# JonathanLehner/korali

Measured on AMD Instinct MI355X. Metric: CMA-ES generations/sec + samples/sec, 128-dim Rosenbrock λ=4096, 1→8 GPUs, higher is better.
Workload: dtype f64; 1 GPU; C2: CMA-ES, 128-dim negative Rosenbrock, lambda=4096, mu=2048 Logarithmic, x0=0, sigma0=1, seed 1337; one experiment per GPU; population=4096, variables=128, covariance_update=exact, parallelism=replicas1

## Files before the change

### korali_amd/csrc/kg_cmaes.hip

```cpp
#include <cmath>
#include <cstdio>
#include <cstdlib>
#include <cstring>
#include <map>
#include <string>
#include <tuple>
#include <vector>

#include "../../include/korali_amd.h"
#include "kg_common.hpp"
#include "kg_chains.hpp"
#include "kg_eigen.hpp"
#include "kg_rng.hpp"
#include <chrono>

namespace kg {


struct CmaesScalars {
  double sigma, trace, effectiveMu, cumulativeCovariance, sigmaCumulationFactor, dampFactor, chiSquareNumber;
  double psNorm, bestEverValue, previousBestEverValue, previousBestValue, currentBestValue;
  double currentMinStd, currentMaxStd, maxDiagC, minDiagC, minEig, maxEig;
  double infeasibleSampleCount, bestValidSample, modelEvaluationCount, hsig, eigenFailures;
  double ccov1, ccovmu;
// ... 1141 lines not shown
    tile[r][tx] = t;
  }
  if (k0 == 0 && ty == 0 && d0 + tx < N) prevMean[d0 + tx] = md;
  __syncthreads();
  for (int r = ty; r < RP_T; r += 8) {
    const int d = d0 + r, k = k0 + tx;
    if (d < N && k < mu) Tt[(size_t)d * mu + k] = tile[tx][r];
  }
  if (__syncthreads_or(!ok) && threadIdx.x == 0) atomicOr(&sc->rmuOutOfRange, 1u);
  if (blockIdx.x || blockIdx.y) return;
  __shared__ int flag;
  if (threadIdx.x == 0) {
    const unsigned i0 = sidx[0];
    sc->bestValidSample = (double)i0;
    sc->previousBestValue = sc->currentBestValue;
    sc->currentBestValue = F[i0];
    flag = (sc->currentBestValue > sc->bestEverValue || gen == 1) ? 1 : 0;
    sc->bestFlag = (unsigned)flag;
    if (flag) {
      sc->previousBestEverValue = sc->bestEverValue;
      sc->bestEverValue = sc->currentBestValue;
    }
  }
  __syncthreads();
  const unsigned i0 = sidx[0];
  for (int d = threadIdx.x; d < N; d += blockDim.x) {
    const double v = X[(size_t)i0 * N + d];
    currBestVars[d] = v;
    if (flag) bestEverVars[d] = v;
  }
}

constexpr int RS_U = 8;
__global__ void __launch_bounds__(256) k_rank_select(int lam, int N, int mu, unsigned long long gen,
                                                     const double *__restrict__ F, unsigned *__restrict__ out,
                                                     const double *__restrict__ X, const double *__restrict__ w,
                                                     const double *__restrict__ mean, double *__restrict__ prevMean,
                                                     double *__restrict__ Y, double *__restrict__ currBestVars,
                                                     double *__restrict__ bestEverVars, CmaesScalars *sc,
                                                     double *__restrict__ Yc, double *__restrict__ Tt) {
  extern __shared__ __attribute__((aligned(16))) double rk[];
  __shared__ unsigned part[16][17];
  __shared__ unsigned rank_s[16];
  __shared__ int flag;
  const int row = threadIdx.x >> 4, c = threadIdx.x & 15;
  const int is = blockIdx.x * 16 + row;
  double xv[RS_U], mv[RS_U];
#pragma unroll
  for (int u = 0; u < RS_U; u++) {
    const int d = c + 16 * u;
    xv[u] = (is < lam && d < N) ? X[(size_t)is * N + d] : 0.0;
    mv[u] = d < N ? mean[d] : 0.0;
  }
  const double effMu = sc->effectiveMu, ca = N + 1.3, cb = N + 2.0;
  const double ccov1 = 2.0 / (ca * ca + effMu);
  double ccovmu = 2.0 * (effMu - 2. + 1. / effMu) / (cb * cb + effMu);
  if (1.0 - ccov1 < ccovmu) ccovmu = 1.0 - ccov1;
  for (int q0 = threadIdx.x; q0 < lam; q0 += 8 * blockDim.x) {
    double v[8];
#pragma unroll
    for (int u = 0; u < 8; u++) v[u] = (q0 + u * (int)blockDim.x < lam) ? F[q0 + u * blockDim.x] : 0.0;
#pragma unroll
    for (int u = 0; u < 8; u++)
      if (q0 + u * (int)blockDim.x < lam) rk[q0 + u * blockDim.x] = v[u];
  }
  if (blockIdx.x == 0)
// ... 5 lines not shown
    const double ki = (i < lam) ? rk[i] : 0.0;
    const int per = (lam + 15) / 16, j0 = p * per, j1 = min(lam, j0 + per);
    unsigned cnt = 0;
    int j = j0;
    for (; j + 8 <= j1; j += 8) {
      double kj[8];
#pragma unroll
      for (int u = 0; u < 8; u++) kj[u] = rk[j + u];
#pragma unroll
      for (int u = 0; u < 8; u++) cnt += (kj[u] > ki || (kj[u] == ki && j + u < i)) ? 1u : 0u;
    }
    for (; j < j1; j++) {
      const double kj = rk[j];
      cnt += (kj > ki || (kj == ki && j < i)) ? 1u : 0u;
    }
    part[p][li] = cnt;
  }
  __syncthreads();
  if (threadIdx.x < 16) {
    unsigned r = 0;
    for (int q = 0; q < 16; q++) r += part[q][threadIdx.x];
    rank_s[threadIdx.x] = r;
    if (blockIdx.x * 16 + (int)threadIdx.x < lam) out[r] = (unsigned)(blockIdx.x * 16 + threadIdx.x);
  }
  __syncthreads();
  const unsigned r = rank_s[row];
  const bool sel = is < lam && r < (unsigned)mu;
  bool ok = true;
  if (sel) {
    const double cw = ccovmu * w[r];
    auto put = [&](int d, double x, double m) {
      Y[(size_t)r * N + d] = x;
      const double yc = x - m;
      Yc[(size_t)r * N + d] = yc;
      const double t = cw * yc;
      Tt[(size_t)d * mu + r] = t;
      ok = ok && rmu_in_range(yc) && rmu_in_range(t);
    };
#pragma unroll
    for (int u = 0; u < RS_U; u++)
      if (c + 16 * u < N) put(c + 16 * u, xv[u], mv[u]);
    for (int d = c + 16 * RS_U; d < N; d += 16) put(d, X[(size_t)is * N + d], mean[d]);
  }
  if (__syncthreads_or(!ok) && threadIdx.x == 0) atomicOr(&sc->rmuOutOfRange, 1u);
  const bool best = is < lam && r == 0u;
  if (!__syncthreads_or(best)) return;
  if (best && c == 0) {
    sc->bestValidSample = (double)is;
    sc->previousBestValue = sc->currentBestValue;
    sc->currentBestValue = rk[is];
    const int fl = (sc->currentBestValue > sc->bestEverValue || gen == 1) ? 1 : 0;
    flag = fl;
    sc->bestFlag = (unsigned)fl;
    if (fl) {
      sc->previousBestEverValue = sc->bestEverValue;
      sc->bestEverValue = sc->currentBestValue;
    }
  }
  __syncthreads();
  if (best) {
    const int fl = flag;
#pragma unroll
    for (int u = 0; u < RS_U; u++) {
      const int d = c + 16 * u;
      if (d < N) {
        currBestVars[d] = xv[u];
        if (fl) bestEverVars[d] = xv[u];
      }
    }
// ... 241 lines not shown
  const bool active = wid == 0 && d < N && e < N && e <= d && (!diagonal || e == d);
  const double ccov1 = sc->ccov1, ccovmu = sc->ccovmu, cc = sc->cumulativeCovariance;
  const int hsig = (int)sc->hsig;
  const double s2 = sc->sigma * sc->sigma;
  double c = 0.0;
  if (active) {
    const double Cde = C[(size_t)d * N + e];
    c = (1 - ccov1 - ccovmu) * Cde + ccov1 * (pc[d] * pc[e] + (1 - hsig) * cc * (2. - cc) * Cde);
  }
  const int ex = (int)((__double_as_longlong(s2) >> 52) & 0x7ff) - 1023;
  if (__builtin_amdgcn_readfirstlane((int)(sc->rmuOutOfRange == 0u && ex >= -100 && ex <= 100)))
    c = ax3_run<true>(c, Yc, Tt, N, mu, d0, e0, wid, lane, s2, 1.0 / s2, Q);
  else
    c = ax3_run<false>(c, Yc, Tt, N, mu, d0, e0, wid, lane, s2, 0.0, Q);
  if (active) {
    C[(size_t)d * N + e] = c;
    if (e < d) C[(size_t)e * N + d] = c;
  }
}

#ifndef KG_AR_TC
#define KG_AR_TC 4
#endif
constexpr int AR_TC = KG_AR_TC, AR_NT = 64 * AR_TC, AR_K = 256, AR_KS = AR_K + 2, AR_TU = 4 * AR_K / AR_NT,
              AR_YU = AR_TC * AR_K / AR_NT;
static_assert(AR_TC == 4 || AR_TC == 8, "4 x 4 or 4 x 8 tiles");
__host__ __device__ inline int ar_row_blocks(int N) { return (N + 3) / 4; }
__host__ __device__ inline int ar_col_blocks_upto(int rb) { return (4 * rb + 3) / AR_TC + 1; }
int ar_tiles(int N) {
  int t = 0;
  for (int rb = 0; rb < ar_row_blocks(N); rb++) t += std::min(ar_col_blocks_upto(rb), (N + AR_TC - 1) / AR_TC);
  return t;
}
template <bool kMarkstein>
__device__ __forceinline__ double ar_run(double acc, int N, int mu, int d0, int e0, int dl, int el,
                                         const double *__restrict__ Yc, const double *__restrict__ Tt, double s2,
                                         double (*Ts)[4][AR_KS], double (*Ys)[AR_TC][AR_KS]) {
  const int tid = threadIdx.x, j = tid & 15;
  const double y = kMarkstein ? 1.0 / s2 : 0.0;
  double tv[AR_TU], yv[AR_YU];
  auto load = [&](int k0) {
#pragma unroll
    for (int u = 0; u < AR_TU; u++) {
      const int q = tid + AR_NT * u, r = q / AR_K;
      int kq = q % AR_K;
      asm volatile("" : "+v"(kq));
      const int k = k0 + kq;
      tv[u] = (d0 + r < N && k < mu) ? Tt[(size_t)(d0 + r) * mu + k] : 0.0;
    }
#pragma unroll
    for (int u = 0; u < AR_YU; u++) {
      const int q = tid + AR_NT * u, k = k0 + q / AR_TC, c = q % AR_TC;
      yv[u] = (k < mu && e0 + c < N) ? Yc[(size_t)k * N + e0 + c] : 0.0;
    }
  };
  auto store = [&](int b) {
#pragma unroll
    for (int u = 0; u < AR_TU; u++) {
      const int q = tid + AR_NT * u;
      int kq = q % AR_K;
      asm volatile("" : "+v"(kq));
      Ts[b][q / AR_K][kq] = tv[u];
    }
#pragma unroll
    for (int u = 0; u < AR_YU; u++) {
      const int q = tid + AR_NT * u;
      Ys[b][q % AR_TC][q / AR_TC] = yv[u];
    }
  };
  load(0);
  store(0);
  __syncthreads();
  for (int k0 = 0, b = 0; k0 < mu; k0 += AR_K, b ^= 1) {
    const bool more = k0 + AR_K < mu;
    if (more) load(k0 + AR_K);
    const int gn = (min(AR_K, mu - k0) + 15) >> 4;
    for (int g = 0; g < gn; g++) {
      const double pr = Ts[b][dl][16 * g + j] * Ys[b][el][16 * g + j];
      double q;
      if (kMarkstein) {
        const double q0 = pr * y;
        const double r = __builtin_fma(-q0, s2, pr);
        q = __builtin_fma(r, y, q0);
      } else {
        q = pr / s2;
      }
      acc = chains::kc_row16(acc, q);
    }
    if (more) store(b ^ 1);
    __syncthreads();
  }
  return acc;
}
__global__ void __launch_bounds__(AR_NT) k_adaptC_row(int N, int mu, int diagonal, const double *__restrict__ Yc,
                                                    const double *__restrict__ Tt, const double *__restrict__ pc,
                                                    double *C, const CmaesScalars *__restrict__ sc, int tbase,
                                                    double *__restrict__ pack) {
  __shared__ double Ts[2][4][AR_KS];
  __shared__ double Ys[2][AR_TC][AR_KS];
  const int tid = threadIdx.x, lane = tid & 63, wid = tid >> 6;
  const int row = lane >> 4, j = lane & 15;
  int t = blockIdx.x + tbase, rb = 0;
  const int ncb = (N + AR_TC - 1) / AR_TC;
  for (;; rb++) {
    const int c = min(ar_col_blocks_upto(rb), ncb);
    if (t < c) break;
    t -= c;
  }
  const int d0 = 4 * rb, e0 = AR_TC * t;
  const int dl = wid / (AR_TC / 4), el = 4 * (wid % (AR_TC / 4)) + row;
  const int d = d0 + dl, e = e0 + el;
  const bool active = d < N && e < N && e <= d && (!diagonal || e == d);
  const double ccov1 = sc->ccov1, ccovmu = sc->ccovmu, cc = sc->cumulativeCovariance;
  const int hsig = (int)sc->hsig;
  const double s2 = sc->sigma * sc->sigma;
  double acc = 0.0;
  if (active) {
    const double Cde = C[(size_t)d * N + e];
    acc = (1 - ccov1 - ccovmu) * Cde + ccov1 * (pc[d] * pc[e] + (1 - hsig) * cc * (2. - cc) * Cde);
  }
  const int ex = (int)((__double_as_longlong(s2) >> 52) & 0x7ff) - 1023;
  if (__builtin_amdgcn_readfirstlane((int)(sc->rmuOutOfRange == 0u && ex >= -100 && ex <= 100)))
    acc = ar_run<true>(acc, N, mu, d0, e0, dl, el, Yc, Tt, s2, Ts, Ys);
  else
    acc = ar_run<false>(acc, N, mu, d0, e0, dl, el, Yc, Tt, s2, Ts, Ys);
  if (pack) {
    if (j == 0 && d < N && e <= d) pack[(size_t)d * (d + 1) / 2 + e] = active ? acc : C[(size_t)d * N + e];
    return;
  }
  if (active && j == 0) {
    C[(size_t)d * N + e] = acc;
    if (e < d) C[(size_t)e * N + d] = acc;
  }
}

#ifndef KG_AL_K
#define KG_AL_K 64
#endif
constexpr int AL_T = 16, AL_K = KG_AL_K, AL_KP = AL_K + 2;
static_assert(AL_K % 2 == 0, "two terms per ds_read_b128");
__host__ __device__ inline int al_blocks(int N) { return (N + AL_T - 1) / AL_T; }
int al_tiles(int N) { return al_blocks(N) * (al_blocks(N) + 1) / 2; }
template <bool kMarkstein>
__device__ __forceinline__ void al_run(int N, int mu, int diagonal, const double *__restrict__ Yc,
                                       const double *__restrict__ Tt, const double *__restrict__ pc, double *C,
                                       const CmaesScalars *__restrict__ sc, int tbase, double *__restrict__ pack,
                                       double (*Ts)[AL_T][AL_KP], double (*Ys)[AL_T][AL_KP]) {
  const int tid = threadIdx.x, dl = tid >> 4, el = tid & 15;
  int t = blockIdx.x + tbase, bd = 0;
  while (t > bd) t -= ++bd;
  const int d0 = AL_T * bd, e0 = AL_T * t;
  const int d = d0 + dl, e = e0 + el;
  const bool active = d < N && e <= d && (!diagonal || e == d);
  const double ccov1 = sc->ccov1, ccovmu = sc->ccovmu, cc = sc->cumulativeCovariance;
  const int hsig = (int)sc->hsig;
  const double s2 = sc->sigma * sc->sigma, y = kMarkstein ? 1.0 / s2 : 0.0;
  double acc = 0.0;
  if (active) {
// ... 172 lines not shown
        const bool ok = e < MN_D * MN2_R && i < mu && c < nd;
        wv[u] = ok ? w[i] : 0.0;
        yv[u] = ok ? Y[(size_t)i * N + d0 + c] : 0.0;
      }
#pragma unroll
      for (int u = 0; u < 8; u++) {
        const int e = e0 + u * nt, r = e >> 3, c = e & 7;
        if (e < MN_D * MN2_R) b[(size_t)c * MN2_RS + r] = wv[u] * yv[u];
      }
    }
  };
  stage(0, tid, 256);
  __syncthreads();
  double acc = 0.0;
  const int c = lane < nd ? lane : 0;
  for (int ch = 0; ch < nchunks; ch++) {
    if (wid == 0) {
      const int rn = min(MN2_R, mu - ch * MN2_R);
      const double *b = pbuf + (size_t)(ch & 1) * MN_D * MN2_RS + (size_t)c * MN2_RS;
      acc = chains::kc_add(acc, lds_addr(b), __builtin_amdgcn_readfirstlane((unsigned)(rn + 15) >> 4));
    } else if (ch + 1 < nchunks) {
      stage(ch + 1, tid - 64, 192);
    }
    __syncthreads();
  }
  if (wid == 0 && lane < nd) {
    const int d = d0 + lane;
    const double prev = prevMean[d];
    mean[d] = acc;
    meanUpdate[d] = (acc - prev) / sc->sigma;
  }
}

constexpr int MR_K = 256, MR_KS = MR_K + 2, MR_U = MR_K * 16 / 256;
constexpr int PR_T = 1024;
template <bool kWait>
__device__ void paths3_body(int N, unsigned long long gen, const double *__restrict__ B, const double *__restrict__ D,
                            const double *meanUpdate, double *auxBDZ, double *ps, double *pc, CmaesScalars *sc,
                            unsigned *arrived, unsigned target);
template <bool kPaths>
__global__ void __launch_bounds__(kPaths ? PR_T : 256)
    k_mean3(int N, int mu, const double *__restrict__ Y, const double *__restrict__ w, double *mean,
            const double *__restrict__ prevMean, double *meanUpdate, CmaesScalars *sc, unsigned long long gen,
            const double *__restrict__ B, const double *__restrict__ D, double *auxBDZ, double *ps, double *pc,
            unsigned *arrived, unsigned target) {
  if (kPaths) {
    if (blockIdx.x == gridDim.x - 1) {
      paths3_body<true>(N, gen, B, D, meanUpdate, auxBDZ, ps, pc, sc, arrived, target);
      return;
    }
    if (threadIdx.x >= 256) return;
  }
  __shared__ double ys[2][16][MR_KS];
  __shared__ double ws[2][MR_K];
  const int tid = threadIdx.x, lane = tid & 63, wid = tid >> 6;
  const int row = lane >> 4, j = lane & 15, dl = 4 * wid + row;
  const int d0 = blockIdx.x * 16;
  const int nch = (mu + MR_K - 1) / MR_K;
  const double pmd = (j == 0 && d0 + dl < N) ? prevMean[d0 + dl] : 0.0, sig = sc->sigma;
  double ld[MR_U], wl = 0.0;
  auto load = [&](int ch) {
#pragma unroll
    for (int u = 0; u < MR_U; u++) {
      const int q = tid + 256 * u, k = q >> 4, c = q & 15, i = ch * MR_K + k;
      ld[u] = (i < mu && d0 + c < N) ? Y[(size_t)i * N + d0 + c] : 0.0;
    }
    const int i = ch * MR_K + tid;
    wl = (tid < MR_K && i < mu) ? w[i] : 0.0;
  };
  auto store = [&](int b) {
#pragma unroll
    for (int u = 0; u < MR_U; u++) {
      const int q = tid + 256 * u, k = q >> 4, c = q & 15;
      ys[b][c][k] = ld[u];
    }
    if (tid < MR_K) ws[b][tid] = wl;
  };
  load(0);
  store(0);
  __syncthreads();
  double acc = 0.0;
  for (int ch = 0; ch < nch; ch++) {
    const int b = ch & 1;
    if (ch + 1 < nch) load(ch + 1);
    const int gn = min(MR_K, mu - ch * MR_K + 15) >> 4;
    for (int g = 0; g < gn; g++) {
      const double q = ws[b][16 * g + j] * ys[b][dl][16 * g + j];
      acc = chains::kc_row16(acc, q);
    }
    if (ch + 1 < nch) store(b ^ 1);
    __syncthreads();
  }
  const int d = d0 + dl;
  if (j == 0 && d < N) {
    mean[d] = acc;
    meanUpdate[d] = (acc - pmd) / sig;
    if (kPaths) __builtin_amdgcn_fence(__ATOMIC_RELEASE, "agent");
  }
  if (kPaths) {
    __syncthreads();
    if (tid == 0) __hip_atomic_fetch_add(arrived, 1u, __ATOMIC_RELAXED, __HIP_MEMORY_SCOPE_AGENT);
  }
}

template <bool kWait>
__device__ __forceinline__ void paths3_body(int N, unsigned long long gen, const double *__restrict__ B,
                                            const double *__restrict__ D, const double *meanUpdate, double *auxBDZ,
                                            double *ps, double *pc, CmaesScalars *sc, unsigned *arrived,
                                            unsigned target) {
  __shared__ double mu_s[128 + 16], aux_s[128 + 16], pn_s[128 + 16];
  __shared__ int hs;
  const int tid = threadIdx.x, lane = tid & 63, wid = tid >> 6;
  const int row = lane >> 4, j = lane & 15;
  const double cs = sc->sigmaCumulationFactor, effMu = sc->effectiveMu, cc = sc->cumulativeCovariance;
  const double chi = sc->chiSquareNumber, hpGen = sc->hsigPowGen, hpCs = sc->hsigPowCs, hp = sc->hsigPow;
  const double pcq = tid < N ? pc[tid] : 0.0;
  double muq = (!kWait && tid < N) ? meanUpdate[tid] : 0.0;
  double Dd[2], psd[2];
#pragma unroll
  for (int p = 0; p < 2; p++) {
    const int d = 64 * p + 4 * wid + row;
    Dd[p] = (j == 0 && d < N) ? D[d] : 1.0;
    psd[p] = (j == 0 && d < N) ? ps[d] : 0.0;
  }
// ... 826 lines not shown
  double *Yc = nullptr, *Tt = nullptr;
  double *dzT = nullptr;
  size_t dzTRows = 0;
  int trW = 0;
  EigenSolver eig;
  int *infeas = nullptr, *assign = nullptr;
  int *selEnd = nullptr;
  unsigned long long *blockEnd = nullptr, *usedBlocks = nullptr;
  bool stateDirty = true;
  size_t resamplingRounds = 0;
  bool mirrored = false;
  double *G = nullptr;
  bool hasDiscrete = false;
  double *gran = nullptr, *mask = nullptr, *maskSigma = nullptr, *ubuf = nullptr, *dzero = nullptr;
  unsigned long long *uused = nullptr;
  size_t ucap = 0;
  size_t blocks = 0;
  int kslices = 8;
  int shards = 1, shardRank = 0, r0 = 0, r1 = 0;
  bool replSample = false;
  int *kidx = nullptr, *shardCnt = nullptr;
  double *part = nullptr;
  int *shardPos = nullptr, *shardCounts = nullptr;
  double *rows = nullptr, *covPack = nullptr;
  size_t rowsCap = 0;
  int rowBlock = -1;
  unsigned long long *eigTrace = nullptr;
  TermSummary *summary = nullptr, *summaryDev = nullptr;
  unsigned long long updates = 0;
  bool sampleBegun = false;
  bool consumePending = false;
  bool fusedSel = true, earlyPub = true;
  bool fusedDraw = true;
  unsigned *meanArrived = nullptr;
  unsigned meanTarget = 0;
  MtStream normal, uniform;
  bool profile = false;
  std::vector<std::tuple<std::string, hipEvent_t, hipEvent_t>> pending;
  std::map<std::string, hipEvent_t> openMarks;
  std::map<std::string, std::pair<double, size_t>> prof;
};

namespace {

struct Stage {
  kg_cmaes_s *h;
  std::string name;
  hipEvent_t a = nullptr, b = nullptr;
  hipStream_t s;
  Stage(kg_cmaes_s *h_, const char *n, hipStream_t on = nullptr) : h(h_), name(n), s(on ? on : h_->stream) {
    if (h->profile) {
      (void)hipEventCreate(&a);
      (void)hipEventCreate(&b);
      (void)hipEventRecord(a, s);
    }
  }
  ~Stage() {
    if (h->profile) {
      (void)hipEventRecord(b, s);
      h->pending.emplace_back(name, a, b);
    }
  }
};

int flush_consume(kg_cmaes_s *h) {
  if (!h->consumePending) return 0;
// ... 322 lines not shown
          dalloc_q(&h->pairCnt, h->nc * (size_t)L) | dalloc_q(&h->listDev, L);
    h->cEval.assign(h->nc * (size_t)L, 0.0);
    h->cInd.assign(h->nc * (size_t)L, 0.0);
    h->cCnt.assign(L, 0.0);
    h->vBounds.assign(h->nc, 0.0);
    h->bestCEval.assign(h->nc, 0.0);
  }
  rc |= dalloc_q(&h->kidx, h->muMax) | dalloc_q(&h->shardCnt, 1) | dalloc_q(&h->part, 2 * (size_t)N + (size_t)(nt * (nt + 1) / 2) * 256);
  if (cfg->shard_count >= 1 && cfg->cov_mode != KG_COV_MFMA) {
    h->rowsCap = h->replSample ? 0 : (size_t)std::min(h->muMax, L / h->shards);
    rc |= dalloc_q(&h->shardPos, h->muMax) | dalloc_q(&h->shardCounts, h->shards + 1) |
          dalloc_q(&h->covPack, (size_t)N * (N + 1) / 2);
    if (h->rowsCap) rc |= dalloc_q(&h->rows, (size_t)h->shards * h->rowsCap * N);
  }
  if (!rc && hipStreamSynchronize(nullptr) != hipSuccess) {
    set_error("kg_cmaes_create: zero fills of the device buffers failed");
    rc = 1;
  }
  if (rc) {
    delete h;
    return 1;
  }
  clk.mark("buffers");
  if (getenv("KORALI_AMD_TRACE_EIGEN")) rc |= dalloc(&h->eigTrace, 32 + 8 * (size_t)std::max(N, 128));
  if (host_alloc(&h->summary, sizeof(TermSummary), hipHostMallocCoherent | hipHostMallocMapped) != hipSuccess ||
      hipHostGetDevicePointer((void **)&h->summaryDev, h->summary, 0) != hipSuccess) {
    delete h;
    KG_CHECK(false, "hipHostMalloc of the termination summary failed");
  }
  memset(h->summary, 0, sizeof(TermSummary));
  if (L <= RANK_MAX && (size_t)L * sizeof(double) > 64 * 1024)
  {
    KG_HIP(allow_dynamic_lds((const void *)k_rank_sort, (int)((size_t)L * sizeof(double))));
    KG_HIP(allow_dynamic_lds((const void *)k_rank_select, (int)((size_t)L * sizeof(double))));
  }
  {
    const size_t pbytes = ((size_t)N * (PA_EC + 1) + N) * sizeof(double);
    if (pbytes > 64 * 1024)
      KG_HIP(allow_dynamic_lds((const void *)k_paths, (int)pbytes));
    KG_HIP(allow_dynamic_lds((const void *)k_mean2, (int)mean2_lds_bytes()));
    if (N <= 128)
      KG_HIP(allow_dynamic_lds((const void *)k_objective2, (int)ob2_lds_bytes(N)));
    if (N <= 128)
      KG_HIP(allow_dynamic_lds((const void *)k_paths2, (int)paths2_lds_bytes(N)));
  }
  if (rc) {
    delete h;
    return 1;
  }
  KG_HIP(stream_acquire(&h->stream));
  KG_HIP(stream_acquire(&h->stream2));
  KG_HIP(hipEventCreateWithFlags(&h->evY, hipEventDisableTiming));
  KG_HIP(hipEventCreateWithFlags(&h->evC, hipEventDisableTiming));
  {
    const char *ev = getenv("KORALI_AMD_EIGEN_CHASE");
    bool hostChase = !cfg->eigen_device_chase;
    if (ev && std::string(ev) == "device") hostChase = false;
    if (ev && std::string(ev) == "host") hostChase = true;
    if (h->eig.init(N, hostChase)) {
      delete h;
      return 1;
    }
  }
  clk.mark("eigen");
  {
    const char *e = getenv("KORALI_AMD_FUSED_SELECT");
    h->fusedSel = !(e && *e == '0');
    e = getenv("KORALI_AMD_EARLY_PUBLISH");
    h->earlyPub = !(e && *e == '0');
    e = getenv("KORALI_AMD_FUSED_DRAW");
    h->fusedDraw = !(e && *e == '0');
  }
  if (set_current(h, h->lamCfg, h->muCfg)) return 1;
  KG_HIP(hipMemcpy(h->lb, lb.data(), N * sizeof(double), hipMemcpyHostToDevice));
  KG_HIP(hipMemcpy(h->ub, ub.data(), N * sizeof(double), hipMemcpyHostToDevice));
  KG_HIP(hipMemcpy(h->iv, iv.data(), N * sizeof(double), hipMemcpyHostToDevice));
  KG_HIP(hipMemcpy(h->istd, istd.data(), N * sizeof(double), hipMemcpyHostToDevice));
  KG_HIP(hipMemcpy(h->minstd, minstd.data(), N * sizeof(double), hipMemcpyHostToDevice));
  KG_HIP(hipMemcpy(h->gran, gran.data(), N * sizeof(double), hipMemcpyHostToDevice));
  KG_HIP(hipMemset(h->mask, 0, N * sizeof(double)));
  KG_HIP(hipMemset(h->maskSigma, 0, N * sizeof(double)));
  const size_t words = h->normal.words_for_normals(rows * N);
  if (h->normal.init(3 * words + 4096) || h->uniform.init(std::max<size_t>(1 << 16, 2 * h->ucap + 4096))) {
    delete h;
    return 1;
  }
  clk.mark("rng_init");
  unsigned char st[5000];
  gsl_seed_state(cfg->normal_seed, st);
  if (h->normal.import_gsl(st, h->stream)) return 1;
  clk.mark("normal_seed");
  gsl_seed_state(cfg->uniform_seed, st);
  if (h->uniform.import_gsl(st, h->stream)) return 1;
  clk.mark("uniform_seed");
  *out = h;
  return 0;
}

int kg_cmaes_destroy(kg_cmaes_t h) {
  if (!h) return 0;
  (void)flush_consume(h);
  (void)hipStreamSynchronize(h->stream);
  if (h->stream2) (void)hipStreamSynchronize(h->stream2);
  h->eig.drain();
// ... 378 lines not shown
  const int N = h->N, mu = h->mu;
  {
    Stage st(h, "sigma");
    if (h->hasDiscrete)
      hipLaunchKernelGGL(k_discrete_masks, dim3(1), dim3(64), 0, h->stream, N, h->lam, h->gran, h->C, h->mask,
                         h->maskSigma, h->sc);
    hipLaunchKernelGGL(k_sigma, dim3(1), dim3(256), 0, h->stream, N, mu, h->cfg.is_sigma_bounded, h->C, h->F, h->idx,
                       h->minstd, h->sc, h->normal.state(), h->uniform.state(), h->summaryDev, ++h->updates,
                       h->hasDiscrete ? h->maskSigma : (const double *)nullptr, h->ps, h->mean, h->muCfg,
                       h->viability ? 1 : 0, h->cfg.target_success_rate, h->cfg.global_success_learning_rate,
                       (unsigned long long)(gen + 1));
    h->stateDirty = false;
    KG_HIP(hipGetLastError());
  }
  return 0;
}


static bool lane_chains(int N) {
  static const int from = [] {
    const char *e = getenv("KORALI_AMD_ADAPTC_LANE_MIN");
    return e && *e ? atoi(e) : 256;
  }();
  return N >= from;
}
static bool row_chains() {
  static const bool on = [] {
    const char *e = getenv("KORALI_AMD_ROWCHAINS");
    return !(e && *e == '0');
  }();
  return on;
}

static void launch_mean3(kg_cmaes_t h) {
  hipLaunchKernelGGL(k_mean3<false>, dim3((h->N + 15) / 16), dim3(256), 0, h->stream, h->N, h->mu, h->Y, h->w, h->mean,
                     h->prevMean, h->meanUpdate, h->sc, 0ULL, (const double *)nullptr, (const double *)nullptr,
                     (double *)nullptr, (double *)nullptr, (double *)nullptr, (unsigned *)nullptr, 0u);
}

static int cmaes_paths(kg_cmaes_t h, size_t generation) {
  const int N = h->N;
  if (N <= 128 && !h->cfg.diagonal_covariance && row_chains()) {
    hipLaunchKernelGGL(k_paths3, dim3(1), dim3(PR_T), 0, h->stream, N, (unsigned long long)generation, h->B, h->D,
                       h->meanUpdate, h->auxBDZ, h->ps, h->pc, h->sc);
    KG_HIP(hipGetLastError());
    return 0;
  }
  if (N <= 128 && !h->cfg.diagonal_covariance) {
    hipLaunchKernelGGL(k_paths2, dim3(1), dim3(256), paths2_lds_bytes(N), h->stream, N, (unsigned long long)generation,
                       h->B, h->D, h->meanUpdate, h->auxBDZ, h->ps, h->pc, h->sc);
    KG_HIP(hipGetLastError());
    return 0;
  }
  const size_t pbytes = ((size_t)N * (PA_EC + 1) + N) * sizeof(double);
  hipLaunchKernelGGL(k_paths, dim3(1), dim3(N <= 1024 ? ((N + 63) / 64) * 64 : 1024), pbytes, h->stream, N,
                     h->cfg.diagonal_covariance, (unsigned long long)generation, h->B, h->D, h->meanUpdate,
                     h->auxBDZ, h->ps, h->pc, h->sc);
  KG_HIP(hipGetLastError());
  return 0;
}


static int ccm_eval(kg_cmaes_t h, const std::vector<size_t> &ids, bool mean, std::vector<double> &out) {
  KG_CHECK(h->cfn, "constraints configured but kg_cmaes_set_constraints was not called");
  const size_t N = h->N, rows = mean ? 1 : ids.size();
  std::vector<double> X(rows * N);
  if (mean) {
    KG_HIP(hipMemcpyAsync(X.data(), h->mean, N * sizeof(double), hipMemcpyDeviceToHost, h->stream));
  } else {
    for (size_t r = 0; r < rows; r++)
// ... 153 lines not shown
  if (hs.bestFlag)
    for (size_t c = 0; c < nc; c++) h->bestCEval[c] = h->cEval[c * S + (size_t)hs.bestValidSample];
  if (h->viability)
    for (size_t c = 0; c < nc; c++) {
      double maxviolation = 0.0;
      for (int i = 0; i < h->mu; ++i)
        if (h->cEval[c * S + idx[i]] > maxviolation) maxviolation = h->cEval[c * S + idx[i]];
      const double t = 0.5 * (maxviolation + h->vBounds[c]);
      const double mn = (t < h->vBounds[c]) ? t : h->vBounds[c];
      h->vBounds[c] = (0.0 < mn) ? mn : 0.0;
    }
  return 0;
}

static bool early_publish_on(kg_cmaes_t h) {
  return h->earlyPub && !h->nc && h->eig.host_tridiag() && !h->cfg.diagonal_covariance;
}
static int early_publish(kg_cmaes_t h) {
  if (!early_publish_on(h)) return 0;
  h->eig.trace = h->eigTrace;
  return h->eig.run_begin(h->C, 0, h->B, h->D, &h->sc->minEig, &h->sc->maxEig, &h->sc->eigenFailures, &h->sc->errors,
                          h->stream, eig_prof, h);
}

static bool fused_select(kg_cmaes_t h) {
  const bool ccm = h->nc > 0 && !h->viability;
  return h->fusedSel && !ccm && h->nc == 0 && h->cfg.mu_type != KG_MU_PROPORTIONAL &&
         h->cfg.cov_mode != KG_COV_MFMA && h->updates > 0;
}
static bool plain_update(kg_cmaes_t h) {
  return h->shards == 1 && fused_select(h) && early_publish_on(h) && row_chains() && h->lam > 256 &&
         h->lam <= RANK_MAX;
}

int kg_cmaes_update(kg_cmaes_t h, size_t generation) {
  KG_CHECK(h->shards == 1, "a population-sharded handle updates through kg_cmaes_update_partial / _finalize");
  const int N = h->N, mu = h->mu;
  const bool ccm = h->nc > 0 && !h->viability;
  const bool fused = fused_select(h);
  const bool plain = plain_update(h);
  if (plain) {
    Stage st(h, "sort");
    hipLaunchKernelGGL(k_rank_select, dim3((h->lam + 15) / 16), dim3(256), (size_t)h->lam * sizeof(double), h->stream,
                       h->lam, N, mu, (unsigned long long)generation, h->F, h->idx, h->X, h->w, h->mean, h->prevMean,
                       h->Y, h->currBestVars, h->bestEverVars, h->sc, h->Yc, h->Tt);
    KG_HIP(hipGetLastError());
  } else if (cmaes_sort(h)) {
    return 1;
  }
  {
    Stage st(h, "mean_paths");
    if (ccm) {
      std::vector<int> viol(h->lam);
      for (int i = 0; i < h->lam; i++) viol[i] = h->cCnt[i] > 0 ? 1 : 0;
      KG_HIP(hipMemcpyAsync(h->violDev, viol.data(), h->lam * sizeof(int), hipMemcpyHostToDevice, h->stream));
      KG_HIP(hipStreamSynchronize(h->stream));
    }
    if (plain) {
    } else if (fused) {
      hipLaunchKernelGGL(k_select_prep, dim3((mu + RP_T - 1) / RP_T, (N + RP_T - 1) / RP_T), dim3(256), 0, h->stream,
                         N, mu, (unsigned long long)generation, h->X, h->F, h->idx, h->w, h->mean, h->prevMean, h->Y,
                         h->currBestVars, h->bestEverVars, h->sc, h->Yc, h->Tt);
      KG_HIP(hipGetLastError());
    } else {
    hipLaunchKernelGGL(k_update_best, dim3(1), dim3(256), 0, h->stream, N, mu, h->cfg.mu_type,
                       (unsigned long long)generation, h->X, h->F, h->idx, h->w, h->currBestVars, h->bestEverVars,
                       h->sc, ccm ? (const int *)h->violDev : (const int *)nullptr, h->lam);
    hipLaunchKernelGGL(k_gather_selected, dim3(mu), dim3(128), 0, h->stream, N, mu, h->X, h->idx, h->Y, h->mean,
                       h->prevMean);
    }
    if (h->cfg.cov_mode == KG_COV_MFMA) {
      KG_HIP(hipEventRecord(h->evY, h->stream));
      KG_HIP(hipStreamWaitEvent(h->stream2, h->evY, 0));
      Stage st(h, "rankmu_mfma", h->stream2);
      hipLaunchKernelGGL(k_rankmu_tile<false>, dim3(rankmu_grid(N, h->kslices)), dim3(256), 0, h->stream2, N, mu,
                         (const int *)nullptr, h->kslices, h->Y, (const int *)nullptr, h->w, h->prevMean, h->sc,
                         h->covPart);
      KG_HIP(hipGetLastError());
      KG_HIP(hipEventRecord(h->evC, h->stream2));
    } else if (!fused) {
      hipLaunchKernelGGL(k_rankmu_prep, dim3((mu + RP_T - 1) / RP_T, (N + RP_T - 1) / RP_T), dim3(256), 0,
                         h->stream, N, mu, h->Y, h->w, h->prevMean, h->sc, h->Yc, h->Tt);
      KG_HIP(hipGetLastError());
    }
    if (plain && N <= 128 && !h->G) {
      const int nMean = (N + 15) / 16;
      unsigned target = h->meanTarget + (unsigned)nMean;
      int n = N, m = mu;
      unsigned long long gen = (unsigned long long)generation;
      void *args[] = {&n,   &m,    &h->Y, &h->w,      &h->mean, &h->prevMean, &h->meanUpdate,  &h->sc,
                      &gen, &h->B, &h->D, &h->auxBDZ, &h->ps,   &h->pc,       &h->meanArrived, &target};
      KG_HIP(launch_resident((const void *)k_mean3<true>, dim3(nMean + 1), dim3(PR_T), args, 0, h->stream, true));
      h->meanTarget = target;
    } else {
      if (row_chains())
        launch_mean3(h);
      else
        hipLaunchKernelGGL(k_mean2, dim3((N + MN_D - 1) / MN_D), dim3(256), mean2_lds_bytes(), h->stream, N, mu,
                           h->Y, h->w, h->mean, h->prevMean, h->meanUpdate, h->sc);
      if (h->G)
        hipLaunchKernelGGL(k_mean_gradient, dim3((N + 63) / 64), dim3(64), 0, h->stream, N, mu,
                           h->cfg.gradient_step_size, h->G, h->idx, h->w, h->mean, h->prevMean, h->meanUpdate, h->sc);
      if (cmaes_paths(h, generation)) return 1;
    }
  }
  {
    Stage st(h, "covariance");
    const int nt = (N + 15) / 16, ntiles = nt * (nt + 1) / 2;
    if (h->cfg.cov_mode == KG_COV_MFMA) {
      KG_HIP(hipStreamWaitEvent(h->stream, h->evC, 0));
      hipLaunchKernelGGL(k_adaptC_combine, dim3(ntiles), dim3(256), 0, h->stream, N, h->kslices, ntiles,
                         h->cfg.diagonal_covariance, h->covPart, h->pc, h->C, h->sc, 0);
    } else {
      static const bool old2 = getenv("KORALI_AMD_ADAPTC2") != nullptr;
      if (!old2 && lane_chains(N)) {
        hipLaunchKernelGGL(k_adaptC_lane, dim3(al_tiles(N)), dim3(256), 0, h->stream, N, mu,
                           h->cfg.diagonal_covariance, h->Yc, h->Tt, h->pc, h->C, h->sc, 0, (double *)nullptr);
      } else if (!old2 && row_chains()) {
        hipLaunchKernelGGL(k_adaptC_row, dim3(ar_tiles(N)), dim3(AR_NT), 0, h->stream, N, mu,
                           h->cfg.diagonal_covariance, h->Yc, h->Tt, h->pc, h->C, h->sc, 0, (double *)nullptr);
      } else if (old2)
        hipLaunchKernelGGL(k_adaptC_exact2, dim3((N + 3) / 4, (N + 63) / 64), dim3(256), 0, h->stream, N, mu,
                           h->cfg.diagonal_covariance, h->Yc, h->Tt, h->pc, h->C, h->sc);
      else
        hipLaunchKernelGGL(k_adaptC_exact3, dim3(ax3_slots(N)), dim3(64 * (AX3_P + 1)), 0, h->stream, N, mu,
                           h->cfg.diagonal_covariance, h->Yc, h->Tt, h->pc, h->C, h->sc);
    }
    KG_HIP(hipGetLastError());
  }
  if (early_publish(h)) return 1;
  if (flush_consume(h)) return 1;
  if (cmaes_sigma(h, generation)) return 1;
  return h->nc ? ccm_after_update(h) : 0;
}

int kg_cmaes_update_partial(kg_cmaes_t h, size_t generation) {
  const int N = h->N, mu = h->mu;
  if (cmaes_sort(h)) return 1;
  if (h->covPack) {
    Stage st(h, "mean_paths");
    const int per = h->lam / h->shards;
    hipLaunchKernelGGL(k_update_best, dim3(1), dim3(256), 0, h->stream, N, mu, h->cfg.mu_type,
                       (unsigned long long)generation, (const double *)nullptr, h->F, h->idx, h->w, h->currBestVars,
                       h->bestEverVars, h->sc, (const int *)nullptr, h->lam);
    if (h->rows) {
      hipLaunchKernelGGL(k_shard_positions, dim3(1), dim3(1024), 0, h->stream, mu, per, h->shards, h->idx, h->shardPos,
                         h->shardCounts);
      hipLaunchKernelGGL(k_shard_pack, dim3(mu), dim3(128), 0, h->stream, N, h->shardRank, per, h->shards, h->idx,
                         h->shardPos, h->shardCounts, h->X, h->rows);
    }
    KG_HIP(hipGetLastError());
    h->rowBlock = -1;
    return 0;
// ... 43 lines not shown
  KG_CHECK(h->rowBlock >= 0, "kg_cmaes_update_rows before kg_cmaes_shard_row_count");
  const int N = h->N, mu = h->mu;
  const int per = h->lam / h->shards;
  {
    Stage st(h, "mean_paths");
    hipLaunchKernelGGL(k_shard_unpack, dim3(mu), dim3(128), 0, h->stream, N, per, h->shards, h->idx, h->shardPos,
                       h->shardCounts, (const double *)h->rows, h->X, h->Y, h->mean, h->prevMean, h->currBestVars,
                       h->bestEverVars, h->sc);
    hipLaunchKernelGGL(k_rankmu_prep, dim3((mu + RP_T - 1) / RP_T, (N + RP_T - 1) / RP_T), dim3(256), 0, h->stream, N,
                       mu, h->Y, h->w, h->prevMean, h->sc, h->Yc, h->Tt);
    if (row_chains())
      launch_mean3(h);
    else
      hipLaunchKernelGGL(k_mean2, dim3((N + MN_D - 1) / MN_D), dim3(256), mean2_lds_bytes(), h->stream, N, mu, h->Y,
                         h->w, h->mean, h->prevMean, h->meanUpdate, h->sc);
    if (h->G)
      hipLaunchKernelGGL(k_mean_gradient, dim3((N + 63) / 64), dim3(64), 0, h->stream, N, mu, h->cfg.gradient_step_size,
                         h->G, h->idx, h->w, h->mean, h->prevMean, h->meanUpdate, h->sc);
    KG_HIP(hipGetLastError());
    if (cmaes_paths(h, generation)) return 1;
  }
  {
    Stage st(h, "covariance");
    const size_t npk = (size_t)N * (N + 1) / 2;
    hipLaunchKernelGGL(k_fill_min_i64, dim3((unsigned)std::min<size_t>((npk + 255) / 256, 1024)), dim3(256), 0,
                       h->stream, npk, (long long *)h->covPack);
    const bool lane = lane_chains(N);
    const int nt = lane ? al_tiles(N) : ar_tiles(N);
    const int t0 = (int)((long long)nt * h->shardRank / h->shards), t1 = (int)((long long)nt * (h->shardRank + 1) / h->shards);
    if (t1 > t0 && lane)
      hipLaunchKernelGGL(k_adaptC_lane, dim3(t1 - t0), dim3(256), 0, h->stream, N, mu, h->cfg.diagonal_covariance,
                         h->Yc, h->Tt, h->pc, h->C, h->sc, t0, h->covPack);
    else if (t1 > t0)
      hipLaunchKernelGGL(k_adaptC_row, dim3(t1 - t0), dim3(AR_NT), 0, h->stream, N, mu, h->cfg.diagonal_covariance, h->Yc,
                         h->Tt, h->pc, h->C, h->sc, t0, h->covPack);
    KG_HIP(hipGetLastError());
  }
  h->rowBlock = -1;
  return 0;
}

int kg_cmaes_update_finalize(kg_cmaes_t h, size_t generation) {
  const int N = h->N;
  if (h->covPack) {
    Stage st(h, "covariance");
    hipLaunchKernelGGL(k_shard_cov_unpack, dim3(N), dim3(256), 0, h->stream, N, (const double *)h->covPack, h->C);
    KG_HIP(hipGetLastError());
    if (early_publish(h)) return 1;
    if (flush_consume(h)) return 1;
    return cmaes_sigma(h, generation);
  }
  {
    Stage st(h, "mean_paths");
    hipLaunchKernelGGL(k_shard_finalize, dim3((N + 255) / 256), dim3(256), 0, h->stream, N, h->part, h->mean,
                       h->prevMean, h->meanUpdate, h->currBestVars, h->bestEverVars, h->sc);
    if (h->G)
      hipLaunchKernelGGL(k_mean_gradient, dim3((N + 63) / 64), dim3(64), 0, h->stream, N, h->mu,
                         h->cfg.gradient_step_size, h->G, h->idx, h->w, h->mean, h->prevMean, h->meanUpdate, h->sc);
    KG_HIP(hipGetLastError());
    if (cmaes_paths(h, generation)) return 1;
  }
  {
    Stage st(h, "covariance");
    const int nt = (N + 15) / 16, ntiles = nt * (nt + 1) / 2;
    hipLaunchKernelGGL(k_adaptC_combine, dim3(ntiles), dim3(256), 0, h->stream, N, 1, ntiles,
                       h->cfg.diagonal_covariance, h->part + 2 * (size_t)N, h->pc, h->C, h->sc, 1);
    KG_HIP(hipGetLastError());
  }
// ... 307 lines not shown
```

Before: 1978 generations/s.

## Derive rank-mu factors inside covariance kernel from transposed Y instead of storing Yc/Tt

Rank-select no longer writes the centred Yc and weighted transposed Tt arrays when the derive path is enabled. Instead, spare blocks in the mean kernel transpose Y into the Tt buffer, and the covariance row kernel rebuilds yc = y - prevMean and t = ccovmu*w*yc on the fly while filling shared memory. It also recomputes ccovmu from effectiveMu on the device. Separately, the mean kernel's chunk prefetch is generalised to a configurable look-ahead depth, which defaults to the old depth of one. The aim is to cut the strided scattered Tt writes and the extra global traffic, at the cost of more complex kernels and a duplicated coefficient formula that must match the host's.

```diff
diff --git a/korali_amd/csrc/kg_cmaes.hip b/korali_amd/csrc/kg_cmaes.hip
--- a/korali_amd/csrc/kg_cmaes.hip
+++ b/korali_amd/csrc/kg_cmaes.hip
@@ -1197,6 +1197,7 @@
 }
 
 constexpr int RS_U = 8;
+template <bool kFactors>
 __global__ void __launch_bounds__(256) k_rank_select(int lam, int N, int mu, unsigned long long gen,
                                                      const double *__restrict__ F, unsigned *__restrict__ out,
                                                      const double *__restrict__ X, const double *__restrict__ w,
@@ -1268,9 +1269,9 @@
     auto put = [&](int d, double x, double m) {
       Y[(size_t)r * N + d] = x;
       const double yc = x - m;
-      Yc[(size_t)r * N + d] = yc;
+      if (kFactors) Yc[(size_t)r * N + d] = yc;
       const double t = cw * yc;
-      Tt[(size_t)d * mu + r] = t;
+      if (kFactors) Tt[(size_t)d * mu + r] = t;
       ok = ok && rmu_in_range(yc) && rmu_in_range(t);
     };
 #pragma unroll
@@ -1578,14 +1579,37 @@
   for (int rb = 0; rb < ar_row_blocks(N); rb++) t += std::min(ar_col_blocks_upto(rb), (N + AR_TC - 1) / AR_TC);
   return t;
 }
-template <bool kMarkstein>
+template <bool kMarkstein, bool kDerive>
 __device__ __forceinline__ double ar_run(double acc, int N, int mu, int d0, int e0, int dl, int el,
                                          const double *__restrict__ Yc, const double *__restrict__ Tt, double s2,
-                                         double (*Ts)[4][AR_KS], double (*Ys)[AR_TC][AR_KS]) {
+                                         double (*Ts)[4][AR_KS], double (*Ys)[AR_TC][AR_KS],
+                                         const double *__restrict__ w, double ccovmu) {
   const int tid = threadIdx.x, j = tid & 15;
   const double y = kMarkstein ? 1.0 / s2 : 0.0;
-  double tv[AR_TU], yv[AR_YU];
+  double tv[AR_TU], yv[AR_YU], wq = 0.0;
+  double mdv[AR_TU], mev[AR_YU];
+  int kt = tid % AR_K;
+  asm volatile("" : "+v"(kt));
+#pragma unroll
+  for (int u = 0; u < AR_TU; u++) mdv[u] = (kDerive && d0 + (tid + AR_NT * u) / AR_K < N) ? Tt[d0 + (tid + AR_NT * u) / AR_K] : 0.0;
+#pragma unroll
+  for (int u = 0; u < AR_YU; u++) mev[u] = (kDerive && e0 + (tid + AR_NT * u) / AR_K < N) ? Tt[e0 + (tid + AR_NT * u) / AR_K] : 0.0;
   auto load = [&](int k0) {
+    if (kDerive) {
+      const int k = k0 + kt;
+#pragma unroll
+      for (int u = 0; u < AR_TU; u++) {
+        const int r = (tid + AR_NT * u) / AR_K;
+        tv[u] = (d0 + r < N && k < mu) ? Yc[(size_t)(d0 + r) * mu + k] : 0.0;
+      }
+#pragma unroll
+      for (int u = 0; u < AR_YU; u++) {
+        const int r = (tid + AR_NT * u) / AR_K;
+        yv[u] = (e0 + r < N && k < mu) ? Yc[(size_t)(e0 + r) * mu + k] : 0.0;
+      }
+      wq = k < mu ? w[k] : 0.0;
+      return;
+    }
 #pragma unroll
     for (int u = 0; u < AR_TU; u++) {
       const int q = tid + AR_NT * u, r = q / AR_K;
@@ -1600,7 +1624,29 @@
       yv[u] = (k < mu && e0 + c < N) ? Yc[(size_t)k * N + e0 + c] : 0.0;
     }
   };
-  auto store = [&](int b) {
+  auto derive = [&](int b, int k0, auto full) {
+    const bool in = full.value || k0 + kt < mu;
+    const double cw = ccovmu * wq;
+#pragma unroll
+    for (int u = 0; u < AR_TU; u++) {
+      const double yc = tv[u] - mdv[u];
+      const double t = cw * yc;
+      Ts[b][(tid + AR_NT * u) / AR_K][kt] = in ? t : 0.0;
+    }
+#pragma unroll
+    for (int u = 0; u < AR_YU; u++) {
+      const double yc = yv[u] - mev[u];
+      Ys[b][(tid + AR_NT * u) / AR_K][kt] = in ? yc : 0.0;
+    }
+  };
+  auto store = [&](int b, int k0) {
+    if (kDerive) {
+      if (k0 + AR_K <= mu)
+        derive(b, k0, std::true_type());
+      else
+        derive(b, k0, std::false_type());
+      return;
+    }
 #pragma unroll
     for (int u = 0; u < AR_TU; u++) {
       const int q = tid + AR_NT * u;
@@ -1615,7 +1661,7 @@
     }
   };
   load(0);
-  store(0);
+  store(0, 0);
   __syncthreads();
   for (int k0 = 0, b = 0; k0 < mu; k0 += AR_K, b ^= 1) {
     const bool more = k0 + AR_K < mu;
@@ -1633,15 +1679,16 @@
       }
       acc = chains::kc_row16(acc, q);
     }
-    if (more) store(b ^ 1);
+    if (more) store(b ^ 1, k0 + AR_K);
     __syncthreads();
   }
   return acc;
 }
+template <bool kDerive>
 __global__ void __launch_bounds__(AR_NT) k_adaptC_row(int N, int mu, int diagonal, const double *__restrict__ Yc,
                                                     const double *__restrict__ Tt, const double *__restrict__ pc,
                                                     double *C, const CmaesScalars *__restrict__ sc, int tbase,
-                                                    double *__restrict__ pack) {
+                                                    double *__restrict__ pack, const double *__restrict__ w) {
   __shared__ double Ts[2][4][AR_KS];
   __shared__ double Ys[2][AR_TC][AR_KS];
   const int tid = threadIdx.x, lane = tid & 63, wid = tid >> 6;
@@ -1666,10 +1713,17 @@
     acc = (1 - ccov1 - ccovmu) * Cde + ccov1 * (pc[d] * pc[e] + (1 - hsig) * cc * (2. - cc) * Cde);
   }
   const int ex = (int)((__double_as_longlong(s2) >> 52) & 0x7ff) - 1023;
+  double cmu = 0.0;
+  if (kDerive) {
+    const double effMu = sc->effectiveMu, ca = N + 1.3, cb = N + 2.0;
+    const double c1 = 2.0 / (ca * ca + effMu);
+    cmu = 2.0 * (effMu - 2. + 1. / effMu) / (cb * cb + effMu);
+    if (1.0 - c1 < cmu) cmu = 1.0 - c1;
+  }
   if (__builtin_amdgcn_readfirstlane((int)(sc->rmuOutOfRange == 0u && ex >= -100 && ex <= 100)))
-    acc = ar_run<true>(acc, N, mu, d0, e0, dl, el, Yc, Tt, s2, Ts, Ys);
+    acc = ar_run<true, kDerive>(acc, N, mu, d0, e0, dl, el, Yc, Tt, s2, Ts, Ys, w, cmu);
   else
-    acc = ar_run<false>(acc, N, mu, d0, e0, dl, el, Yc, Tt, s2, Ts, Ys);
+    acc = ar_run<false, kDerive>(acc, N, mu, d0, e0, dl, el, Yc, Tt, s2, Ts, Ys, w, cmu);
   if (pack) {
     if (j == 0 && d < N && e <= d) pack[(size_t)d * (d + 1) / 2 + e] = active ? acc : C[(size_t)d * N + e];
     return;
@@ -1908,24 +1962,50 @@
   }
 }
 
-constexpr int MR_K = 256, MR_KS = MR_K + 2, MR_U = MR_K * 16 / 256;
+#ifndef KG_MR_AHEAD
+#define KG_MR_AHEAD 1
+#endif
+constexpr int MR_K = 256, MR_KS = MR_K + 2, MR_U = MR_K * 16 / 256, MR_AHEAD = KG_MR_AHEAD;
+static_assert(MR_AHEAD >= 1 && MR_AHEAD <= 3, "chunks in flight: 32 VGPRs each, 128 in all for k_mean3<true>");
 constexpr int PR_T = 1024;
 template <bool kWait>
 __device__ void paths3_body(int N, unsigned long long gen, const double *__restrict__ B, const double *__restrict__ D,
                             const double *meanUpdate, double *auxBDZ, double *ps, double *pc, CmaesScalars *sc,
                             unsigned *arrived, unsigned target);
-template <bool kPaths>
+template <bool kPaths, bool kYt>
 __global__ void __launch_bounds__(kPaths ? PR_T : 256)
     k_mean3(int N, int mu, const double *__restrict__ Y, const double *__restrict__ w, double *mean,
             const double *__restrict__ prevMean, double *meanUpdate, CmaesScalars *sc, unsigned long long gen,
             const double *__restrict__ B, const double *__restrict__ D, double *auxBDZ, double *ps, double *pc,
-            unsigned *arrived, unsigned target) {
+            unsigned *arrived, unsigned target, double *__restrict__ Yt) {
   if (kPaths) {
     if (blockIdx.x == gridDim.x - 1) {
       paths3_body<true>(N, gen, B, D, meanUpdate, auxBDZ, ps, pc, sc, arrived, target);
       return;
     }
     if (threadIdx.x >= 256) return;
+  }
+  if (kYt && (int)blockIdx.x >= (N + 15) / 16) {
+    __shared__ double tl[32][33];
+    const int first = (N + 15) / 16, nT = (int)gridDim.x - first - (kPaths ? 1 : 0);
+    const int tx = threadIdx.x & 31, ty = threadIdx.x >> 5;
+    const int td = (N + 31) / 32, tiles = ((mu + 31) / 32) * td;
+    for (int t = (int)blockIdx.x - first; t < tiles; t += nT) {
+      const int k0 = (t / td) * 32, c0 = (t % td) * 32;
+#pragma unroll
+      for (int r = 0; r < 4; r++) {
+        const int k = k0 + ty + 8 * r, d = c0 + tx;
+        tl[ty + 8 * r][tx] = (k < mu && d < N) ? Y[(size_t)k * N + d] : 0.0;
+      }
+      __syncthreads();
+#pragma unroll
+      for (int r = 0; r < 4; r++) {
+        const int d = c0 + ty + 8 * r, k = k0 + tx;
+        if (d < N && k < mu) Yt[(size_t)d * mu + k] = tl[tx][ty + 8 * r];
+      }
+      __syncthreads();
+    }
+    return;
   }
   __shared__ double ys[2][16][MR_KS];
   __shared__ double ws[2][MR_K];
@@ -1934,38 +2014,44 @@
   const int d0 = blockIdx.x * 16;
   const int nch = (mu + MR_K - 1) / MR_K;
   const double pmd = (j == 0 && d0 + dl < N) ? prevMean[d0 + dl] : 0.0, sig = sc->sigma;
-  double ld[MR_U], wl = 0.0;
-  auto load = [&](int ch) {
+  double ld[MR_AHEAD][MR_U], wl[MR_AHEAD];
+  auto load = [&](int ch, double *l, double &wq) {
 #pragma unroll
     for (int u = 0; u < MR_U; u++) {
       const int q = tid + 256 * u, k = q >> 4, c = q & 15, i = ch * MR_K + k;
-      ld[u] = (i < mu && d0 + c < N) ? Y[(size_t)i * N + d0 + c] : 0.0;
+      l[u] = (i < mu && d0 + c < N) ? Y[(size_t)i * N + d0 + c] : 0.0;
     }
     const int i = ch * MR_K + tid;
-    wl = (tid < MR_K && i < mu) ? w[i] : 0.0;
+    wq = (tid < MR_K && i < mu) ? w[i] : 0.0;
   };
-  auto store = [&](int b) {
+  auto store = [&](int b, const double *l, double wq) {
 #pragma unroll
     for (int u = 0; u < MR_U; u++) {
       const int q = tid + 256 * u, k = q >> 4, c = q & 15;
-      ys[b][c][k] = ld[u];
-    }
-    if (tid < MR_K) ws[b][tid] = wl;
+      ys[b][c][k] = l[u];
+    }
+    if (tid < MR_K) ws[b][tid] = wq;
   };
-  load(0);
-  store(0);
+#pragma unroll
+  for (int a = 0; a < MR_AHEAD; a++)
+    if (a < nch) load(a, ld[a], wl[a]);
+  store(0, ld[0], wl[0]);
   __syncthreads();
   double acc = 0.0;
-  for (int ch = 0; ch < nch; ch++) {
-    const int b = ch & 1;
-    if (ch + 1 < nch) load(ch + 1);
-    const int gn = min(MR_K, mu - ch * MR_K + 15) >> 4;
-    for (int g = 0; g < gn; g++) {
-      const double q = ws[b][16 * g + j] * ys[b][dl][16 * g + j];
-      acc = chains::kc_row16(acc, q);
-    }
-    if (ch + 1 < nch) store(b ^ 1);
-    __syncthreads();
+  for (int c0 = 0; c0 < nch; c0 += MR_AHEAD) {
+#pragma unroll
+    for (int s = 0; s < MR_AHEAD; s++) {
+      const int ch = c0 + s, b = ch & 1;
+      if (ch >= nch) break;
+      if (ch + MR_AHEAD < nch) load(ch + MR_AHEAD, ld[s], wl[s]);
+      const int gn = min(MR_K, mu - ch * MR_K + 15) >> 4;
+      for (int g = 0; g < gn; g++) {
+        const double q = ws[b][16 * g + j] * ys[b][dl][16 * g + j];
+        acc = chains::kc_row16(acc, q);
+      }
+      if (ch + 1 < nch) store(b ^ 1, ld[(s + 1) % MR_AHEAD], wl[(s + 1) % MR_AHEAD]);
+      __syncthreads();
+    }
   }
   const int d = d0 + dl;
   if (j == 0 && d < N) {
@@ -2858,6 +2944,7 @@
   bool consumePending = false;
   bool fusedSel = true, earlyPub = true;
   bool fusedDraw = true;
+  bool deriveFac = true;
   unsigned *meanArrived = nullptr;
   unsigned meanTarget = 0;
   MtStream normal, uniform;
@@ -3246,7 +3333,8 @@
   if (L <= RANK_MAX && (size_t)L * sizeof(double) > 64 * 1024)
   {
     KG_HIP(allow_dynamic_lds((const void *)k_rank_sort, (int)((size_t)L * sizeof(double))));
-    KG_HIP(allow_dynamic_lds((const void *)k_rank_select, (int)((size_t)L * sizeof(double))));
+    KG_HIP(allow_dynamic_lds((const void *)k_rank_select<true>, (int)((size_t)L * sizeof(double))));
+    KG_HIP(allow_dynamic_lds((const void *)k_rank_select<false>, (int)((size_t)L * sizeof(double))));
   }
   {
     const size_t pbytes = ((size_t)N * (PA_EC + 1) + N) * sizeof(double);
@@ -3284,6 +3372,8 @@
     h->earlyPub = !(e && *e == '0');
     e = getenv("KORALI_AMD_FUSED_DRAW");
     h->fusedDraw = !(e && *e == '0');
+    e = getenv("KORALI_AMD_DERIVE_FACTORS");
+    h->deriveFac = !(e && *e == '0');
   }
   if (set_current(h, h->lamCfg, h->muCfg)) return 1;
   KG_HIP(hipMemcpy(h->lb, lb.data(), N * sizeof(double), hipMemcpyHostToDevice));
@@ -3728,10 +3818,13 @@
   return on;
 }
 
-static void launch_mean3(kg_cmaes_t h) {
-  hipLaunchKernelGGL(k_mean3<false>, dim3((h->N + 15) / 16), dim3(256), 0, h->stream, h->N, h->mu, h->Y, h->w, h->mean,
+static int mean3_transposers(int N, int mu) { return std::min(64, ((mu + 31) / 32) * ((N + 31) / 32)); }
+static void launch_mean3(kg_cmaes_t h, bool yt = false) {
+  const auto mean3 = yt ? k_mean3<false, true> : k_mean3<false, false>;
+  hipLaunchKernelGGL(mean3, dim3((h->N + 15) / 16 + (yt ? mean3_transposers(h->N, h->mu) : 0)), dim3(256), 0, h->stream, h->N, h->mu, h->Y, h->w, h->mean,
                      h->prevMean, h->meanUpdate, h->sc, 0ULL, (const double *)nullptr, (const double *)nullptr,
-                     (double *)nullptr, (double *)nullptr, (double *)nullptr, (unsigned *)nullptr, 0u);
+                     (double *)nullptr, (double *)nullptr, (double *)nullptr, (unsigned *)nullptr, 0u,
+                     yt ? h->Tt : (double *)nullptr);
 }
 
 static int cmaes_paths(kg_cmaes_t h, size_t generation) {
@@ -3951,16 +4044,24 @@
   return h->shards == 1 && fused_select(h) && early_publish_on(h) && row_chains() && h->lam > 256 &&
          h->lam <= RANK_MAX;
 }
+static bool adaptc2_old() {
+  static const bool old2 = getenv("KORALI_AMD_ADAPTC2") != nullptr;
+  return old2;
+}
+static bool derive_factors(kg_cmaes_t h) {
+  return h->deriveFac && plain_update(h) && !adaptc2_old() && !lane_chains(h->N);
+}
 
 int kg_cmaes_update(kg_cmaes_t h, size_t generation) {
   KG_CHECK(h->shards == 1, "a population-sharded handle updates through kg_cmaes_update_partial / _finalize");
   const int N = h->N, mu = h->mu;
   const bool ccm = h->nc > 0 && !h->viability;
   const bool fused = fused_select(h);
-  const bool plain = plain_update(h);
+  const bool plain = plain_update(h), derive = derive_factors(h);
   if (plain) {
     Stage st(h, "sort");
-    hipLaunchKernelGGL(k_rank_select, dim3((h->lam + 15) / 16), dim3(256), (size_t)h->lam * sizeof(double), h->stream,
+    const auto select = derive ? k_rank_select<false> : k_rank_select<true>;
+    hipLaunchKernelGGL(select, dim3((h->lam + 15) / 16), dim3(256), (size_t)h->lam * sizeof(double), h->stream,
                        h->lam, N, mu, (unsigned long long)generation, h->F, h->idx, h->X, h->w, h->mean, h->prevMean,
                        h->Y, h->currBestVars, h->bestEverVars, h->sc, h->Yc, h->Tt);
     KG_HIP(hipGetLastError());
@@ -4007,13 +4108,16 @@
       unsigned target = h->meanTarget + (unsigned)nMean;
       int n = N, m = mu;
       unsigned long long gen = (unsigned long long)generation;
-      void *args[] = {&n,   &m,    &h->Y, &h->w,      &h->mean, &h->prevMean, &h->meanUpdate,  &h->sc,
-                      &gen, &h->B, &h->D, &h->auxBDZ, &h->ps,   &h->pc,       &h->meanArrived, &target};
-      KG_HIP(launch_resident((const void *)k_mean3<true>, dim3(nMean + 1), dim3(PR_T), args, 0, h->stream, true));
+      double *yt = derive ? h->Tt : nullptr;
+      void *args[] = {&n,   &m,    &h->Y, &h->w,      &h->mean, &h->prevMean, &h->meanUpdate,  &h->sc, &gen,
+                      &h->B, &h->D, &h->auxBDZ, &h->ps,   &h->pc,       &h->meanArrived, &target, &yt};
+      const void *mean3 = derive ? (const void *)k_mean3<true, true> : (const void *)k_mean3<true, false>;
+      const int nYt = derive ? mean3_transposers(N, mu) : 0;
+      KG_HIP(launch_resident(mean3, dim3(nMean + nYt + 1), dim3(PR_T), args, 0, h->stream, true));
       h->meanTarget = target;
     } else {
       if (row_chains())
-        launch_mean3(h);
+        launch_mean3(h, derive);
       else
         hipLaunchKernelGGL(k_mean2, dim3((N + MN_D - 1) / MN_D), dim3(256), mean2_lds_bytes(), h->stream, N, mu,
                            h->Y, h->w, h->mean, h->prevMean, h->meanUpdate, h->sc);
@@ -4031,13 +4135,18 @@
       hipLaunchKernelGGL(k_adaptC_combine, dim3(ntiles), dim3(256), 0, h->stream, N, h->kslices, ntiles,
                          h->cfg.diagonal_covariance, h->covPart, h->pc, h->C, h->sc, 0);
     } else {
-      static const bool old2 = getenv("KORALI_AMD_ADAPTC2") != nullptr;
-      if (!old2 && lane_chains(N)) {
+      const bool old2 = adaptc2_old();
+      if (derive) {
+        hipLaunchKernelGGL(k_adaptC_row<true>, dim3(ar_tiles(N)), dim3(AR_NT), 0, h->stream, N, mu,
+                           h->cfg.diagonal_covariance, h->Tt, h->prevMean, h->pc, h->C, h->sc, 0, (double *)nullptr,
+                           h->w);
+      } else if (!old2 && lane_chains(N)) {
         hipLaunchKernelGGL(k_adaptC_lane, dim3(al_tiles(N)), dim3(256), 0, h->stream, N, mu,
                            h->cfg.diagonal_covariance, h->Yc, h->Tt, h->pc, h->C, h->sc, 0, (double *)nullptr);
       } else if (!old2 && row_chains()) {
-        hipLaunchKernelGGL(k_adaptC_row, dim3(ar_tiles(N)), dim3(AR_NT), 0, h->stream, N, mu,
-                           h->cfg.diagonal_covariance, h->Yc, h->Tt, h->pc, h->C, h->sc, 0, (double *)nullptr);
+        hipLaunchKernelGGL(k_adaptC_row<false>, dim3(ar_tiles(N)), dim3(AR_NT), 0, h->stream, N, mu,
+                           h->cfg.diagonal_covariance, h->Yc, h->Tt, h->pc, h->C, h->sc, 0, (double *)nullptr,
+                           (const double *)nullptr);
       } else if (old2)
         hipLaunchKernelGGL(k_adaptC_exact2, dim3((N + 3) / 4, (N + 63) / 64), dim3(256), 0, h->stream, N, mu,
                            h->cfg.diagonal_covariance, h->Yc, h->Tt, h->pc, h->C, h->sc);
@@ -4147,8 +4256,9 @@
       hipLaunchKernelGGL(k_adaptC_lane, dim3(t1 - t0), dim3(256), 0, h->stream, N, mu, h->cfg.diagonal_covariance,
                          h->Yc, h->Tt, h->pc, h->C, h->sc, t0, h->covPack);
     else if (t1 > t0)
-      hipLaunchKernelGGL(k_adaptC_row, dim3(t1 - t0), dim3(AR_NT), 0, h->stream, N, mu, h->cfg.diagonal_covariance, h->Yc,
-                         h->Tt, h->pc, h->C, h->sc, t0, h->covPack);
+      hipLaunchKernelGGL(k_adaptC_row<false>, dim3(t1 - t0), dim3(AR_NT), 0, h->stream, N, mu,
+                         h->cfg.diagonal_covariance, h->Yc, h->Tt, h->pc, h->C, h->sc, t0, h->covPack,
+                         (const double *)nullptr);
     KG_HIP(hipGetLastError());
   }
   h->rowBlock = -1;
```

Result: slower. 1955 generations/s (-1.2%).
